# mozack/vdjer

Measured on AMD Instinct MI355X. Metric: M paired-reads/sec (k-mer build + contig score), IgH 50bp PE, higher is better.
Workload: dtype u8/u64 (2-bit packed bases, integer counts)

## Files before the change

vdjer_amd/csrc/vdjx_kmer.hip:

```cpp
#include "vdjx_common.h"

#include <algorithm>
#include <numeric>
#include <type_traits>
#include <string.h>
#include <stdlib.h>

#define HIST_THREADS 512
#define HIST_BLOCKS 512u
#define LOCAL_SLOTS 2048u
#define K3_SUB_TUPLES g_sub_tuples
__device__ u32 g_sub_tuples = 262144u;
#define NONE32 0xFFFFFFFFu
#define INST_MASK 0x7FFFFFFFu

struct RecView {
	u64 bhi, blo, nm, lq;
};

__device__ inline RecView load_rec(const u64* __restrict__ bases, const u64* __restrict__ nmask,
                                   const u64* __restrict__ lowq, size_t r) {
	RecView v;
	const ulonglong2 b = ((const ulonglong2*) bases)[r];
	v.bhi = b.x; v.blo = b.y;
// ... 425 lines not shown
	for (u32 i = threadIdx.x; i < nbk; i += 512) h[i] = 0;
	__syncthreads();
	const u32 seg = blockIdx.x / slices, sl = blockIdx.x % slices;
	const size_t s0 = seg_start[(size_t) seg << seg_shift], s1 = seg_start[((size_t) seg + 1) << seg_shift];
	const size_t per = (s1 - s0 + slices - 1) / slices;
	const size_t t0 = s0 + (size_t) sl * per;
	const size_t t1 = t0 + per < s1 ? t0 + per : s1;
	for (size_t t = t0 + threadIdx.x; t < t1; t += 512) {
		const TUP x = TUP::load(&in[t]);
		atomicAdd(&h[(u32) (vdjx_bucket_mix(x.lo, x.hi()) >> shift) & (nbk - 1)], 1u);
	}
	__syncthreads();
	for (u32 i = threadIdx.x; i < nbk; i += 512) if (h[i]) atomicAdd(&fine_cnt[((size_t) seg << sub_bits) | i], h[i]);
}

#ifndef RD_THREADS
#define RD_THREADS 768
#define RD_UNR 4
#define RD_WAVES 6
#endif
#define RD_SLOTS 2048u
#define RD_SLOT_BITS 11
#define RD_PQ 4096u
#define RD_LI 512u
#define RD_LROWS 128u
#define RD_MAXLOW 11u
#define ST_CAND 1u
#define ST_MULTI 2u
#define ST_QOK 4u
#define ST_QOK_R 8u
#define ST_ID_SHIFT 8
#define ST_NOID 0xFFFFFFu

struct SurvOutG { u64* lo; u64* hi; u32* gcnt; u64* gfirst; u32* n; u32 cap; u32* n_real; };
#define GC_SHADOW 0x80000000u
#define GC_MASK 0x7FFFFFFFu

__device__ inline bool reads_equal(const u64* __restrict__ bases, const u64* __restrict__ nmask, int rl, u64 a, u64 b) {
	if (rl <= VDJX_SHORT_READ_LEN) {
		const ulonglong2 x = ((const ulonglong2*) bases)[a];
		const ulonglong2 y = ((const ulonglong2*) bases)[b];
		return x.x == y.x && x.y == y.y && nmask[a] == nmask[b];
	}
	u64 d = 0;
#pragma unroll
	for (int w = 0; w < VDJX_LONG_W; w++) d |= bases[a * VDJX_LONG_W + w] ^ bases[b * VDJX_LONG_W + w];
#pragma unroll
	for (int w = 0; w < VDJX_LONG_M; w++) d |= nmask[a * VDJX_LONG_M + w] ^ nmask[b * VDJX_LONG_M + w];
// ... 28 lines not shown
		}
	}
	if (active) { c0 = atomicAdd(&cnt[idx], 1u); atomicMin((unsigned long long*) &mn[idx], (unsigned long long) val); }
	return c0;
}

__global__ __launch_bounds__(1024) void k_bucket_order(const u32* __restrict__ bucket_start, u32 NB, u32* __restrict__ order) {
	__shared__ u32 cls_cnt[33], cls_at[33];
	if (threadIdx.x < 33) cls_cnt[threadIdx.x] = 0;
	__syncthreads();
	for (u32 b = threadIdx.x; b < NB; b += 1024) {
		const u32 n = bucket_start[b + 1] - bucket_start[b];
		atomicAdd(&cls_cnt[n ? 32u - (u32) __builtin_clz(n) : 0u], 1u);
	}
	__syncthreads();
	if (threadIdx.x == 0) { u32 at = 0; for (int cl = 32; cl >= 0; cl--) { cls_at[cl] = at; at += cls_cnt[cl]; } }
	__syncthreads();
	for (u32 b = threadIdx.x; b < NB; b += 1024) {
		const u32 n = bucket_start[b + 1] - bucket_start[b];
		order[atomicAdd(&cls_at[n ? 32u - (u32) __builtin_clz(n) : 0u], 1u)] = b;
	}
}

template <typename TUP, bool SYM = false>
__global__ __launch_bounds__(RD_THREADS, sizeof(TUP) == 16 ? RD_WAVES : RD_WAVES / 2) void k_gated_reduce(const TUP* __restrict__ tup, const u32* __restrict__ bucket_start,
                                                             const u64* __restrict__ bases, const u64* __restrict__ nmask,
                                                             vdjx_qrows quals, int rl, int ob, int k, u64 rec_base,
                                                             u32 mf, u32 cmin, u32 mqq, u32 tlow, SurvOutG so,
                                                             u64* __restrict__ g_distinct, u32* __restrict__ g_err, u32 dbg_in,
                                                             const u32* __restrict__ order) {
#ifdef VDJX_ABLATE
	const u32 dbg = dbg_in;
#else
	const u32 dbg = dbg_in == 9u ? 9u : 0u;
#endif
	typedef typename TUP::hi_t THI;
	__shared__ u64 s_klo[RD_SLOTS];
	__shared__ THI s_khi[RD_SLOTS];
	__shared__ u64 s_first[RD_SLOTS];
	__shared__ u32 s_cnt[RD_SLOTS], s_state[RD_SLOTS];
	__shared__ u32 pq[RD_PQ];
	__shared__ u64 low_inst[RD_LI];
	__shared__ u32 low_n[RD_LROWS];
	__shared__ unsigned short low_slot[RD_LROWS];
	__shared__ u32 s_over, s_ndist, s_nlow, s_npq, s_nsurv, s_base, s_nreal;
	const THI EMPTY = (THI) ~(THI) 0;
	const u32 b = order ? order[blockIdx.x] : blockIdx.x;
	const u32 base = bucket_start[b];
	const u32 n = bucket_start[b + 1] - base;
	const u32 tid = threadIdx.x;
	if (n == 0) return;
	const TUP* T = tup + base;
	const u32 om = (1u << ob) - 1u;
	const u32 per_low = tlow > 1 ? (tlow - 1 < RD_MAXLOW ? tlow - 1 : RD_MAXLOW) : 1;
	const u32 lrows = RD_LI / per_low < RD_LROWS ? RD_LI / per_low : RD_LROWS;
	u32 S = 1;
	while ((u64) S * K3_SUB_TUPLES < n) S <<= 1;
	u32 ndist_total = 0;
	bool verify = S > 1;
	for (;;) {
		if (tid == 0) { s_over = 0; s_ndist = 0; }
		__syncthreads();
		for (u32 s = 0; s < S; s++) {
			for (u32 i = tid; i < RD_SLOTS; i += RD_THREADS) { s_khi[i] = EMPTY; s_cnt[i] = 0; s_first[i] = NONE64; s_state[i] = 0; }
			if (tid == 0) { s_nlow = 0; s_npq = (n >> (32 - RD_SLOT_BITS) || dbg == 9) ? RD_PQ + 1 : 0; s_nsurv = 0; s_nreal = 0; }
			__syncthreads();
			for (u32 t0 = 0; t0 < n; t0 += RD_UNR * RD_THREADS) {
				TUP r_t[RD_UNR];
#pragma unroll
				for (int j = 0; j < RD_UNR; j++) {
					const u32 t = t0 + j * RD_THREADS + tid;
					if (t < n) r_t[j] = TUP::load(&T[t]);
				}
#pragma unroll
				for (int j = 0; j < RD_UNR; j++) {
					const u32 t = t0 + j * RD_THREADS + tid;
					int slot = -1;
					if (t < n) {
						const u32 h = rd_hash(r_t[j].lo, r_t[j].hi());
						if (!(S > 1 && ((h >> 12) & (S - 1)) != s)) {
							slot = lds_insert<THI, RD_SLOTS>(s_klo, s_khi, r_t[j].lo, (THI) r_t[j].hi(), h);
							if (slot < 0) s_over = 1;
						}
					}
					const bool live = slot >= 0 && !verify;
					const u64 inst = r_t[j].inst();
					const u32 c0 = rd_count_min(s_cnt, s_first, (u32) (live ? slot : 0), inst, live);
					bool list = false;
					if (live) {
						u32 st = vdjx_peek(&s_state[slot]);
						if (!(st & ST_MULTI)) {
							const u64 f = vdjx_peek(&s_first[slot]);
							if (f != NONE64 && (f >> ob) != (inst >> ob)) {
								const u32 o1 = (u32) inst & om, o0 = (u32) f & om;
								const u32 d = o1 > o0 ? o1 - o0 : o0 - o1;
								if (d && d < (u32) k && !vdjx_kmer_has_period(r_t[j].hi(), r_t[j].lo, k, d)) { atomicOr(&s_state[slot], ST_MULTI); st |= ST_MULTI; }
							}
						}
						list = !((st & ST_MULTI) && c0 + 1 >= tlow);
					}
					const u32 qi = vdjx_wave_inc(&s_npq, list);
					if (list && qi < RD_PQ) pq[qi] = (t << RD_SLOT_BITS) | (u32) slot;
				}
			}
			__syncthreads();
			if (s_over || verify) { if (s_over) break; continue; }
			if (dbg == 1) return;
			for (u32 i = tid; i < RD_SLOTS; i += RD_THREADS) {
				if (s_khi[i] == EMPTY) continue;
				atomicAdd(&s_ndist, SYM ? 2u : 1u);
				const u32 c = s_cnt[i];
				if (c >= cmin) s_state[i] = (s_state[i] & ST_MULTI) | ST_CAND | ((c < tlow ? atomicAdd(&s_nlow, 1u) : ST_NOID) << ST_ID_SHIFT);
			}
			__syncthreads();
			const u32 nlow = s_nlow;
			const bool listed = s_npq <= RD_PQ;
			const u32 nscan = listed ? s_npq : n;
			for (u32 l0 = 0; l0 == 0 || l0 < nlow; l0 += lrows) {
				for (u32 i = tid; i < RD_LROWS; i += RD_THREADS) low_n[i] = 0;
				__syncthreads();
				for (u32 e = tid; e < nscan; e += RD_THREADS) {
					u32 slot, t;
					TUP x;
					if (listed) {
						slot = pq[e] & (RD_SLOTS - 1); t = pq[e] >> RD_SLOT_BITS;
						if (!(vdjx_peek(&s_state[slot]) & ST_CAND)) continue;
						x = TUP::load(&T[t]);
					} else {
						x = TUP::load(&T[e]);
						const u32 h = rd_hash(x.lo, x.hi());
						if (S > 1 && ((h >> 12) & (S - 1)) != s) continue;
						const int sl = lds_lookup<THI, RD_SLOTS>(s_klo, s_khi, x.lo, (THI) x.hi(), h);
						if (sl < 0) continue;
						slot = (u32) sl;
					}
					const u32 st = vdjx_peek(&s_state[slot]);
					if (!(st & ST_CAND)) continue;
					const u64 inst = x.inst(), fi = s_first[slot];
					const u32 lid = st >> ST_ID_SHIFT;
					if (lid != ST_NOID && lid >= l0 && lid < l0 + lrows) {
						const u32 pos = atomicAdd(&low_n[lid - l0], 1u);
						if (pos < per_low) low_inst[(lid - l0) * per_low + pos] = inst;
						low_slot[lid - l0] = (unsigned short) slot;
					}
					if (l0 == 0 && !(st & ST_MULTI) && (inst >> ob) != (fi >> ob)) {
						const u32 o1 = (u32) inst & om, o0 = (u32) fi & om;
						const u32 d = o1 > o0 ? o1 - o0 : o0 - o1;
						if ((d && d < (u32) k && !vdjx_kmer_has_period(x.hi(), x.lo, k, d))
						    || !reads_equal(bases, nmask, rl, (inst >> ob) - rec_base, (fi >> ob) - rec_base)) atomicOr(&s_state[slot], ST_MULTI);
					}
				}
				__syncthreads();
				if (dbg == 4) return;
				const u32 rows = nlow - l0 < lrows ? nlow - l0 : lrows;
				const u32 lane = tid & 63u;
				for (u32 r = tid >> 6; r < (nlow ? rows : 0u); r += RD_THREADS / 64) {
					const u32 slot = low_slot[r], cnt = low_n[r];
					const u64 fi = s_first[slot];
					u32 qv[RD_MAXLOW];
#pragma unroll
					for (u32 i = 0; i < RD_MAXLOW; i++) {
						qv[i] = 33u;
						if (i < cnt && i < per_low) {
							const u64 inst = low_inst[r * per_low + i];
							const uint8_t* q = quals.row((inst >> ob) - rec_base) + (inst == fi ? 0u : (u32) inst & om);
							if (lane < (u32) k) qv[i] = q[lane];
						}
					}
					u32 sum = 0;
#pragma unroll
					for (u32 i = 0; i < RD_MAXLOW; i++) sum += (u32) (uint8_t) (qv[i] - 33u);
					const bool lowq = lane < (u32) k && sum < mqq;
					if (!__ballot(lowq) && lane == 0) atomicOr(&s_state[slot], ST_QOK);
					if (SYM) {
						u64 fr = NONE64;
#pragma unroll
						for (u32 i = 0; i < RD_MAXLOW; i++)
							if (i < cnt && i < per_low) { const u64 m = vdjx_inst_mirror(low_inst[r * per_low + i], ob, rl, k); fr = m < fr ? m : fr; }
#pragma unroll
						for (u32 i = 0; i < RD_MAXLOW; i++) {
							qv[i] = 33u;
							if (i < cnt && i < per_low) {
								const u64 inst = vdjx_inst_mirror(low_inst[r * per_low + i], ob, rl, k);
								const uint8_t* q = quals.row((inst >> ob) - rec_base) + (inst == fr ? 0u : (u32) inst & om);
								if (lane < (u32) k) qv[i] = q[lane];
							}
						}
						u32 sum_r = 0;
#pragma unroll
						for (u32 i = 0; i < RD_MAXLOW; i++) sum_r += (u32) (uint8_t) (qv[i] - 33u);
						const bool lowq_r = lane < (u32) k && sum_r < mqq;
						if (!__ballot(lowq_r) && lane == 0) atomicOr(&s_state[slot], ST_QOK_R);
					}
				}
				__syncthreads();
			}
			if (dbg == 5) return;
			for (u32 i = tid; i < RD_SLOTS; i += RD_THREADS) {
				const u32 st = s_state[i];
				bool keep = false, keep_r = false;
				if (st & ST_CAND) {
					const u32 craw = s_cnt[i];
					const u32 c = craw > 32765u ? 32765u : craw;
					keep = c >= mf && (st & ST_MULTI) && (craw >= tlow || (st & ST_QOK));
					if (SYM) keep_r = c >= mf && (st & ST_MULTI) && (craw >= tlow || (st & ST_QOK_R));
				}
				if (SYM) {
					s_state[i] = (keep || keep_r) ? (atomicAdd(&s_nsurv, 2u) << 2) | (u32) keep | ((u32) keep_r << 1) : NONE32;
					if (keep || keep_r) atomicAdd(&s_nreal, (u32) keep + (u32) keep_r);
				} else s_state[i] = keep ? atomicAdd(&s_nsurv, 1u) : NONE32;
			}
			__syncthreads();
			if (tid == 0) { s_base = s_nsurv ? atomicAdd(so.n, s_nsurv) : 0; if (SYM && s_nreal) atomicAdd(so.n_real, s_nreal); }
			__syncthreads();
			for (u32 i = tid; i < RD_SLOTS; i += RD_THREADS) {
				if (s_state[i] == NONE32) continue;
				u32 pos = s_base + (SYM ? s_state[i] >> 2 : s_state[i]);
				const u32 cgo = s_cnt[i] > 32765u ? 32765u : s_cnt[i];
				if (pos < so.cap) {
					so.lo[pos] = s_klo[i];
					so.hi[pos] = (u64) s_khi[i];
					so.gcnt[pos] = cgo | (SYM && !(s_state[i] & 1u) ? GC_SHADOW : 0u);
					so.gfirst[pos] = s_first[i];
				}
				if (SYM) {
					pos += 1u;
					if (pos < so.cap) {
						u64 rh, rlo;
						vdjx_kmer_rc((u64) s_khi[i], s_klo[i], k, rh, rlo);
						so.lo[pos] = rlo;
						so.hi[pos] = rh;
						so.gcnt[pos] = cgo | (!(s_state[i] & 2u) ? GC_SHADOW : 0u);
						so.gfirst[pos] = vdjx_inst_mirror(s_first[i], ob, rl, k);
					}
				}
			}
			__syncthreads();
		}
// ... 545 lines not shown

__global__ void k_node_flags(const u64* __restrict__ s_lo, const u64* __restrict__ s_hi, u32 n, int k,
                             const u32* __restrict__ vbits, const u32* __restrict__ jbits,
                             uint8_t* __restrict__ has_v, uint8_t* __restrict__ has_j) {
	u32 i = blockIdx.x * blockDim.x + threadIdx.x;
	if (i >= n) return;
	if (k <= 16) { has_v[i] = 1; has_j[i] = 1; return; }
	u128 key = ((u128) s_hi[i] << 64) | s_lo[i];
	u32 code = (u32) (key >> (2 * (k - 16)));
	has_v[i] = code ? (vbits[code >> 5] >> (code & 31)) & 1u : 0;
	has_j[i] = code ? (jbits[code >> 5] >> (code & 31)) & 1u : 0;
}


#define IT_INST_BITS 35
#define IT_INST_MASK ((1ull << IT_INST_BITS) - 1ull)
#define IT_SURV_SHIFT 38
int vdjx_sort_pairs_raw(void* tmp, size_t* tmp_bytes, hipStream_t st, u64* k_in, u64* k_out, u32* v_in, u32* v_out, u32 n, unsigned end_bit);
#define IT_HOLE 0xFFFFFFFFFFFFFFFFull
#define WALK_THREADS 256

#define SLOT_HI_BITS 36
#define SLOT_HI_MASK ((1ull << SLOT_HI_BITS) - 1ull)
struct SurvTable { const ulonglong2* slots; u32 mask; const ulonglong2* skey; const u32* bloom; u32 bloom_mask; };

struct ItemFmt {
	u32 pmask;
	u32 len_shift;
	u32 maxlen;
	u32 mul, inv;
	u32 bmask;
	u32 ns;
};
__device__ inline u32 it_surv(const ItemFmt& f, u64 x) { return (u32) (x >> IT_SURV_SHIFT) & f.pmask; }
__device__ inline u32 it_len(const ItemFmt& f, u64 x) { return f.maxlen > 1 ? (u32) (x >> f.len_shift) + 1u : 1u; }
__device__ inline u32 it_scat(const ItemFmt& f, u32 p) { return ((((p >> 4) * f.mul) & f.bmask) << 4) | (p & 15u); }

__global__ void k_surv_table2(const u64* __restrict__ s_lo, const u64* __restrict__ s_hi, u32 n, ulonglong2* __restrict__ slots, u32 mask,
                              ulonglong2* __restrict__ skey, u32* __restrict__ bloom, u32 bloom_mask) {
	const u32 i = blockIdx.x * blockDim.x + threadIdx.x;
	if (i >= n) return;
	const u64 lo = s_lo[i], hi = s_hi[i];
	skey[i] = make_ulonglong2(lo, hi);
	const u64 h = vdjx_mix(lo, hi);
	{
		const u32 bit = (u32) (h >> 40) & bloom_mask;
		atomicOr(&bloom[bit >> 5], 1u << (bit & 31));
	}
	u32 slot = (u32) (h >> 20) & mask;
	const unsigned long long entry = hi | ((unsigned long long) (i + 1) << SLOT_HI_BITS);
	while (atomicCAS((unsigned long long*) &slots[slot].y, 0ull, entry) != 0ull) slot = (slot + 1) & mask;
	slots[slot].x = lo;
}

__device__ inline int surv_lookup2f(const SurvTable& t, u64 lo, u64 hi);

__device__ inline int surv_lookup2(const SurvTable& t, u64 lo, u64 hi) {
	u32 slot = (u32) (vdjx_mix(lo, hi) >> 20) & t.mask;
	for (;;) {
		const ulonglong2 v = t.slots[slot];
		if (!v.y) return -1;
		if (v.x == lo && (v.y & SLOT_HI_MASK) == hi) return (int) (v.y >> SLOT_HI_BITS) - 1;
		slot = (slot + 1) & t.mask;
	}
}

__device__ inline int surv_lookup2f(const SurvTable& t, u64 lo, u64 hi) {
	const u64 h = vdjx_mix(lo, hi);
	const u32 bit = (u32) (h >> 40) & t.bloom_mask;
	if (!((t.bloom[bit >> 5] >> (bit & 31)) & 1u)) return -1;
	return surv_lookup2(t, lo, hi);
}

__global__ void k_succ_links2(SurvTable t, u32 n, int k, const u32* __restrict__ gcnt, u32* __restrict__ succ, unsigned long long* __restrict__ pred,
                              u32* __restrict__ bestsucc) {
	const u32 u = blockIdx.x * blockDim.x + threadIdx.x;
	if (u >= n) return;
	const ulonglong2 kk = t.skey[u];
	const u128 base = (((u128) kk.y << 64) | kk.x) << 2;
	const u128 km = k < 64 ? (((u128) 1) << (2 * k)) - 1 : ~(u128) 0;
	const int sh = 2 * (k - 1);
	const u32 fb = (u32) (sh < 64 ? kk.x >> sh : kk.y >> (sh - 64)) & 3u;
	const unsigned long long mine = ((unsigned long long) (gcnt[u] & GC_MASK) << 32) | ((unsigned long long) (fb ^ 1u) << 30) | (unsigned long long) u;
	u32 best = NONE32, best_g = 0;
	for (u32 b = 0; b < 4; b++) {
		const u128 key = (base | (u128) b) & km;
		const int s = surv_lookup2(t, (u64) key, (u64) (key >> 64));
		succ[u * 4 + b] = s >= 0 ? (u32) s : NONE32;
		if (s >= 0 && (u32) s != u) {
			const u32 g = gcnt[s] & GC_MASK;
			if (best == NONE32 || g >= best_g) { best = (u32) s; best_g = g; }
			atomicMax(&pred[s], mine);
// ... 260 lines not shown
				if (lm) {
					if (later) {
						const u32 qi = qn + (u32) __popcll(lm & ((1ull << lane) - 1ull));
						dq[wq][qi] = ((u64) r << 8) | (u64) (u32) o;
						if constexpr (!LONG) { dq_b[wq][qi] = make_ulonglong2(v.bhi, v.blo); dq_v[wq][qi] = V; }
						o = P; need = false;
					}
					qn += (u32) __popcll(lm);
				}
			}
			WST(if (__ballot(need)) st_lookup++;)
			if (!FRESH && __ballot(need && !first && !have_c)) {
				WST(st_filter++;)
				const bool mine = need && !first && !have_c;
				for (int ob = 0; ob < P; ob += 4) {
					u32 wv[4], bt[4];
#pragma unroll
					for (int j = 0; j < 4; j++) {
						const int oo = ob + j;
						wv[j] = 0; bt[j] = 0;
						if (mine && oo >= o && oo < P && wm_test(V, oo)) {
							u64 khi, klo;
							v.kmer_u(k, oo, khi, klo);
							const u32 bit = (u32) (vdjx_mix(klo, khi) >> 40) & t.bloom_mask;
							bt[j] = bit & 31u;
							wv[j] = (dbg & 8u) ? 0xFFFFFFFFu : t.bloom[bit >> 5];
						}
					}
#pragma unroll
					for (int j = 0; j < 4; j++) if ((wv[j] >> bt[j]) & 1u) wm_set(C, ob + j);
				}
				if (mine) have_c = true;
			}
			if (need) {
				bool filtered = false;
				if (!first) {
					o = wm_next(C, o, P);
					filtered = true;
				}
				first = false;
				if (o < P) {
					u64 khi, klo;
					v.kmer_l(k, o, khi, klo);
					if (dbg & 8u) s = (klo & 3u) ? (int) ((u32) vdjx_mix(klo, khi) % f.ns) : -1;
					else s = (filtered || (dbg & 16u)) ? surv_lookup2(t, klo, khi) : surv_lookup2f(t, klo, khi);
					in = 0;
					if (s < 0) o++;
// ... 473 lines not shown
	for (int e = 0; e < 4; e++) { o.from_ids[(size_t) r * 4 + e] = f[e] != NONE64 ? id[e] : 0; deg += f[e] != NONE64; }
	o.from_deg[r] = (uint8_t) deg;
}

namespace {

struct PersistAlloc {
	vdjx_ctx* c;
	explicit PersistAlloc(vdjx_ctx* ctx) : c(ctx) {}
	template <typename T> hipError_t alloc(T** out, size_t n) {
		*out = (T*) c->shard_arena.alloc((n ? n : 1) * sizeof(T));
		return *out ? hipSuccess : hipErrorOutOfMemory;
	}
	vdjx_arena::mark_t mark() const { return c->shard_arena.mark(); }
	void release_to(vdjx_arena::mark_t m) { c->shard_arena.release_to(m); }
};

struct PoolView { const u64* bases; const u64* nmask; vdjx_qrows quals; int rl; int ob; };

template <typename TUP> struct GTuples {
	TUP* t = nullptr;
	u32* bucket_start = nullptr;
	u32 NB = 0, N = 0;
};

struct SurvivorsG {
	u64 *lo = nullptr, *hi = nullptr, *gfirst = nullptr, *ufirst = nullptr;
	u32 *gcnt = nullptr, *ucnt = nullptr;
	u32 n = 0, n_real = 0;
	u64 ndist = 0;
};

inline u32 ceil_log2_u64(u64 x) { u32 b = 0; while ((1ull << b) < x) b++; return b; }

static bool sync_debug() { static const bool on = vdjx_env_set("VDJX_SYNC_DEBUG"); return on; }
static void dbg_sync(vdjx_ctx* c, const char* what) {
	if (!sync_debug()) return;
	const hipError_t e = hipStreamSynchronize(c->stream);
	fprintf(stderr, "[vdjx] %s: %s\n", what, hipGetErrorString(e));
}

struct GatedHist { u32 HB = 0, NBH = 0, N = 0; u32* hstart = nullptr; bool sym = false; };
static bool build_sym(const vdjx_pool* pool, int k) {
	return pool->sym && pool->W == 2 && (k & 1) && pool->n_records % 2 == 0;
}
static bool sym_walk_wanted() { static const bool on = !vdjx_env_set("VDJX_NO_SYM_WALK"); return on; }
static size_t gated_bucket_default() { static const size_t v = (size_t) vdjx_env_num("VDJX_GATED_BUCKET", 3072, 1, 1ll << 32); return v; }
template <typename A>
int stage_gated_hist(vdjx_ctx* c, A& db, const vdjx_pool* pool, int k, size_t per_bucket, u64 geometry_instances, GatedHist* gh, bool sym = false) {
	hipStream_t st = c->stream;
	const size_t R = sym ? pool->n_records / 2 : pool->n_records;
	const int P = pool->rl - k + 1;
	const u64 NI = geometry_instances ? geometry_instances : (u64) R * (u64) P;
	const size_t per = per_bucket ? per_bucket : gated_bucket_default();
	const u32 hb_max = pool->W > 2 ? 14u : 15u;
	u32 HB = ceil_log2_u64((NI + per - 1) / per);
	HB = std::max(8u, std::min(hb_max, HB));
	const u32 NBH = 1u << HB;
#ifdef VDJX_ABLATE
	static const u32 hist_dbg = (u32) vdjx_env_num("VDJX_HIST_DBG", 0, 0, 4);
#else
	constexpr u32 hist_dbg = 0;
#endif
	u32 nblk = (u32) std::min<size_t>(HIST_BLOCKS, (R + 4095) / 4096);
	if (nblk == 0) nblk = 1;
	size_t rpb = (R + nblk - 1) / nblk;
	u32 *hcnt, *hstart;
	HIP_TRY(db.alloc(&hcnt, NBH));
	HIP_TRY(db.alloc(&hstart, NBH + 1));
	HIP_TRY(hipMemsetAsync(hcnt, 0, (size_t) NBH * 4, st));
	const bool lng = pool->W > 2;
	const size_t lds_hist = (size_t) NBH * 4 + (HIST_THREADS / 64) * (lng ? GL_WAVE_BYTES_LONG : GL_WAVE_BYTES);
	HIP_TRY(hipFuncSetAttribute((const void*) k_gated_hist<false>, hipFuncAttributeMaxDynamicSharedMemorySize, (int) lds_hist));
	HIP_TRY(hipFuncSetAttribute((const void*) k_gated_hist<true>, hipFuncAttributeMaxDynamicSharedMemorySize, (int) lds_hist));
	HIP_TRY(hipFuncSetAttribute((const void*) k_gated_hist<false, true>, hipFuncAttributeMaxDynamicSharedMemorySize, (int) lds_hist));
	{
		vdjx_prof_scope ps(c, "k_gated_hist");
// ... 11 lines not shown
#endif
	const u32 N = *(const u32*) c->h_pin;
	c->stats["gated_instances"] = sym ? 2ull * N : N;
	gh->HB = HB; gh->NBH = NBH; gh->N = N; gh->hstart = hstart; gh->sym = sym;
	return VDJX_OK;
}

template <typename TUP, typename A>
int stage_gated_cut(vdjx_ctx* c, A& db, const vdjx_pool* pool, u64 rec_base, int k, size_t per_bucket, u64 geometry_instances, const GatedHist& gh, GTuples<TUP>* out) {
	hipStream_t st = c->stream;
	const bool sym = gh.sym;
	const size_t R = sym ? pool->n_records / 2 : pool->n_records;
	const int P = pool->rl - k + 1;
	const size_t per = per_bucket ? per_bucket : gated_bucket_default();
	const u32 hb_max = pool->W > 2 ? 14u : 15u;
	const bool lng = pool->W > 2;
	const u32 HB = gh.HB, NBH = gh.NBH, N = gh.N;
	u32* hstart = gh.hstart;
	size_t rpb;
	out->N = N;
	const u64 Ng = geometry_instances ? geometry_instances : (u64) N;
	static const size_t refine = (size_t) vdjx_env_num("VDJX_REFINE_TUPLES", 4096, 1, 1ll << 32);
	u32 T = 8;
	while (T < HB && ((u64) per << T) < Ng) T++;
	u32 extra = 0;
	const size_t refine_at = per_bucket ? std::max<size_t>(per_bucket, refine / 2) : refine;
	if (T == HB && HB == hb_max && Ng / NBH > refine_at) {
		extra = 1;
		while (extra < 5 && (Ng >> extra) / NBH > refine_at) extra++;
	}
	const u32 Tt = T + extra;
	const u32 NBt = 1u << Tt;
	HIP_TRY(db.alloc(&out->t, (size_t) N + 1));
	constexpr u32 stage_tuples = PARTR_STAGE_BYTES / (u32) sizeof(TUP);
	constexpr u32 lds_partr = PARTR_STAGE_BYTES + stage_tuples * 4;
	HIP_TRY(hipFuncSetAttribute((const void*) k_part_records_g<TUP, false>, hipFuncAttributeMaxDynamicSharedMemorySize, (int) lds_partr));
	HIP_TRY(hipFuncSetAttribute((const void*) k_part_records_g<TUP, true>, hipFuncAttributeMaxDynamicSharedMemorySize, (int) lds_partr));
	HIP_TRY(hipFuncSetAttribute((const void*) k_part_records_g<TUP, false, true>, hipFuncAttributeMaxDynamicSharedMemorySize, (int) lds_partr));
	HIP_TRY(hipFuncSetAttribute((const void*) k_part_tuples_g<TUP>, hipFuncAttributeMaxDynamicSharedMemorySize, PART_LDS_BYTES));
	u32 cbits = Tt, fbits = 0;
	if (Tt > 10) { cbits = extra ? Tt - 10 : 8; fbits = Tt - cbits; }
	const u32 NBc = 1u << cbits;
	u32 nblk2 = (u32) std::min<size_t>(1024, (R + 2047) / 2048);
	if (nblk2 == 0) nblk2 = 1;
	rpb = (R + nblk2 - 1) / nblk2;
	u32* gcur;
	HIP_TRY(db.alloc(&gcur, NBc));
	TUP* l1 = out->t;
	if (fbits) HIP_TRY(db.alloc(&l1, (size_t) N + 1));
	{
		vdjx_prof_scope ps(c, "k_part_records");
		hipLaunchKernelGGL(k_init_cursors, dim3((NBc + 255) / 256), dim3(256), 0, st, hstart, NBc, HB - cbits, gcur);
		const u64 NIl = (u64) R * (u64) P;
		u64 rr = N ? (u64) stage_tuples * 3 / 4 * NIl / ((u64) N * (u64) P) : 1u << 16;
// ... 58 lines not shown
}

template <typename TUP, typename A>
int stage_gated_reduce(vdjx_ctx* c, A& db, const GTuples<TUP>& t, const PoolView& pv, u64 rec_base, int k, int mf, int mq, SurvivorsG* sv, bool sym = false) {
	hipStream_t st = c->stream;
	int rc = set_sub_tuples(c);
	if (rc) return rc;
	if (mq >= 255) mq = 254;
	const u32 mqq = (u32) (mq < 0 ? 0 : (mq > 214 ? 214 : mq));
	const u32 tlow = 1 + (mqq + 19) / 20;
	const u32 cmin = (u32) std::max(mf, 2);
	const u32 mfu = (u32) std::max(mf, 0);
	const u32 cap = (sym ? t.N : t.N / 2) + 16;
	u32 *g_err, *n_surv;
	u64* g_distinct;
	HIP_TRY(db.alloc(&sv->lo, cap)); HIP_TRY(db.alloc(&sv->hi, cap)); HIP_TRY(db.alloc(&sv->gcnt, cap)); HIP_TRY(db.alloc(&sv->gfirst, cap));
	HIP_TRY(db.alloc(&g_distinct, 64 * 16 + 2));
	g_err = (u32*) (g_distinct + 64 * 16);
	n_surv = g_err + 1;
	u32* n_real = g_err + 2;
	HIP_TRY(hipMemsetAsync(g_distinct, 0, (64 * 16 + 2) * 8, st));
	SurvOutG so{sv->lo, sv->hi, sv->gcnt, sv->gfirst, n_surv, cap, n_real};
	static const u32 rd_dbg = (u32) vdjx_env_num("VDJX_RD_DBG", 0, 0, 9);
	if (t.N) {
		vdjx_prof_scope ps(c, "k_gated_reduce");
		u32* order;
		if ((rc = bucket_order(c, db, t, &order))) return rc;
		if (sym) hipLaunchKernelGGL((k_gated_reduce<TUP, true>), dim3(t.NB), dim3(RD_THREADS), 0, st, t.t, t.bucket_start, pv.bases, pv.nmask, pv.quals, pv.rl, pv.ob, k, rec_base,
		                            mfu, cmin, mqq, tlow, so, g_distinct, g_err, rd_dbg, (const u32*) order);
		else hipLaunchKernelGGL(k_gated_reduce<TUP>, dim3(t.NB), dim3(RD_THREADS), 0, st, t.t, t.bucket_start, pv.bases, pv.nmask, pv.quals, pv.rl, pv.ob, k, rec_base,
		                        mfu, cmin, mqq, tlow, so, g_distinct, g_err, rd_dbg, (const u32*) order);
	}
	u64* spread = (u64*) c->h_pin;
	u32* tail = (u32*) (spread + 64 * 16);
	static_assert((64 * 16 + 2) * 8 == VDJX_HPIN_SYNC_BYTES, "h_pin layout (vdjx_common.h)");
	HIP_TRY(hipMemcpyAsync(spread, g_distinct, VDJX_HPIN_SYNC_BYTES, hipMemcpyDeviceToHost, st));
	HIP_TRY(hipStreamSynchronize(st));
	HIP_TRY(hipGetLastError());
	const u32 ns = tail[1], err = tail[0];
	if (err) { vdjx_set_error("k_gated_reduce: %u buckets could not be split to fit LDS", err); return VDJX_EHIP; }
	if (ns > cap) { vdjx_set_error("survivor capacity logic failed (%u > %u)", ns, cap); return VDJX_EHIP; }
	sv->ndist = 0;
	for (int i = 0; i < 64; i++) sv->ndist += spread[i * 16];
	sv->n = ns;
	sv->n_real = sym ? tail[2] : ns;
	c->stats["kmer_build_shadows"] = ns - sv->n_real;
	return VDJX_OK;
}

struct RecountOut { u32* ucnt; u64* ufirst; u64* in_first; u32* in_from; u64* edge_first; u32* edge_to; };
struct RecountStatus { const u32* g_err = nullptr; const u32* n_items = nullptr; const unsigned long long* n_inst = nullptr; u32 ns = 0; };
#define VDJX_ESYMWALK (-1000)
static int recount_status_check(vdjx_ctx* c, const u32* hp, u32 ns) {
	if (hp[6] || hp[7]) { vdjx_set_error("the mirrored walk found %u + %u places where the chains are not mirror images", hp[6], hp[7]); return VDJX_ESYMWALK; }
	if (hp[0]) { vdjx_set_error("k_walk_items: item buffer too small (%u waves stopped)", hp[0]); return VDJX_EHIP; }
	if (hp[1]) { vdjx_set_error("internal error: %u of %u surviving k-mers were not met again in the records (VDJX_SYNC_DEBUG=1 names them)", hp[1], ns); return VDJX_EHIP; }
	c->stats["recount_items"] = hp[2];
	c->stats["recount_instances"] = *(const unsigned long long*) (hp + 4);
	return VDJX_OK;
}

template <typename A>
int stage_recount(vdjx_ctx* c, A& db, const vdjx_pool* pool, u64 rec_base, int k, SurvivorsG& sv, const RecountOut& ro,
                  bool derive_edges, SurvTable* table_out = nullptr, RecountStatus* defer = nullptr, bool sym_walk = false) {
	hipStream_t st = c->stream;
	const size_t R = pool->n_records;
	const int P = pool->rl - k + 1;
	const u32 ns = sv.n;
	if (ns >= (1u << 26)) { vdjx_set_error("more than 2^26 surviving k-mers: not supported by the recount items"); return VDJX_ELIMIT; }
	if (R >= (1ull << 29)) { vdjx_set_error("more than 2^29 records on one GPU: not supported by the recount items"); return VDJX_ELIMIT; }
	if ((u64) R * (u64) P >= (1ull << 32)) { vdjx_set_error("records*offsets = %llu >= 2^32 on one GPU: shard the pool over more GPUs", (unsigned long long) ((u64) R * (u64) P)); return VDJX_ELIMIT; }
	u32 tmask = 1023;
	while ((size_t) tmask + 1 < (size_t) ns * 2) tmask = tmask * 2 + 1;
	unsigned long long* pred;
	ulonglong2* table;
	u32 *succ0, *succ, *bloom, *clen, *coff, *csum, *csum_start, *newidx, *jump_open, *fbw, *gcnt2, *bestsucc, *partner = nullptr;
	u64 *pd, *lo2, *hi2, *gfirst2, *linw;
	ulonglong2 *skey0, *skey;
	u32 bloom_bits = 1u << 16;
	while (bloom_bits < (1u << 30) && (size_t) bloom_bits < (size_t) ns * 16) bloom_bits <<= 1;
	const u32 nb16 = (ns + 15u) >> 4;
	const u32 n_scan = (ns + SCAN_BLOCK - 1) / SCAN_BLOCK;
	const u32 n_jump = (ceil_log2_u64((u64) ns + 1) + 4) / 5 + 1;
	{
		auto up = [](size_t b) { return (b + 255) & ~(size_t) 255; };
		const size_t b_bloom = up(bloom_bits / 8), b_table = up(((size_t) tmask + 1) * 16), b_pred = up((size_t) ns * 8), b_clen = up((size_t) ns * 4),
		             b_jump = up((size_t) (n_jump + 1) * 4), b_linw = up(((size_t) nb16 + 1) * 8);
		uint8_t* z;
		const size_t zb = b_bloom + b_table + b_pred + b_clen + b_jump + b_linw;
		HIP_TRY(db.alloc(&z, zb));
		HIP_TRY(hipMemsetAsync(z, 0, zb, st));
		table = (ulonglong2*) z; z += b_table;
		bloom = (u32*) z; z += b_bloom;
		pred = (unsigned long long*) z; z += b_pred;
		clen = (u32*) z; z += b_clen;
		jump_open = (u32*) z; z += b_jump;
		linw = (u64*) z;
	}
	HIP_TRY(db.alloc(&skey0, ns)); HIP_TRY(db.alloc(&skey, ns));
	HIP_TRY(db.alloc(&succ0, (size_t) ns * 4)); HIP_TRY(db.alloc(&succ, (size_t) ns * 4));
	HIP_TRY(db.alloc(&pd, ns)); HIP_TRY(db.alloc(&coff, ns));
	HIP_TRY(db.alloc(&csum, n_scan)); HIP_TRY(db.alloc(&csum_start, n_scan + 1)); HIP_TRY(db.alloc(&newidx, ns));
	HIP_TRY(db.alloc(&lo2, ns)); HIP_TRY(db.alloc(&hi2, ns)); HIP_TRY(db.alloc(&gcnt2, ns)); HIP_TRY(db.alloc(&gfirst2, ns));
	HIP_TRY(db.alloc(&fbw, nb16));
	HIP_TRY(db.alloc(&bestsucc, ns));
	if (sym_walk) HIP_TRY(db.alloc(&partner, ns));
	const SurvTable tb0{table, tmask, skey0, bloom, bloom_bits - 1};
	const SurvTable tb{table, tmask, skey, bloom, bloom_bits - 1};
	if (table_out) *table_out = tb;
	const dim3 gs((ns + 255) / 256), bs(256);
	{
		vdjx_prof_scope ps(c, "k_surv_table");
		hipLaunchKernelGGL(k_surv_table2, gs, bs, 0, st, sv.lo, sv.hi, ns, table, tmask, skey0, bloom, bloom_bits - 1);
		hipLaunchKernelGGL(k_succ_links2, gs, bs, 0, st, tb0, ns, k, sv.gcnt, succ0, pred, bestsucc);
	}
	{
		vdjx_prof_scope ps(c, "k_chain_order");
		hipLaunchKernelGGL(k_chain_init, gs, bs, 0, st, pred, bestsucc, ns, pd);
		for (u32 j = 0; j < n_jump; j++) hipLaunchKernelGGL(k_chain_jump, gs, bs, 0, st, pd, ns, j ? jump_open + j - 1 : (const u32*) nullptr, jump_open + j);
		hipLaunchKernelGGL(k_chain_len, gs, bs, 0, st, pd, ns, clen);
		hipLaunchKernelGGL(k_scan_sums, dim3(n_scan), dim3(256), 0, st, clen, ns, csum);
		hipLaunchKernelGGL(k_bucket_scan, dim3(1), dim3(1024), 0, st, csum, n_scan, csum_start);
		hipLaunchKernelGGL(k_scan_apply, dim3(n_scan), dim3(256), 0, st, clen, ns, csum_start, coff);
		hipLaunchKernelGGL(k_chain_place, gs, bs, 0, st, pd, coff, ns, newidx);
		hipLaunchKernelGGL(k_chain_permute, gs, bs, 0, st, newidx, ns, sv.lo, sv.hi, sv.gcnt, sv.gfirst, succ0, lo2, hi2, gcnt2, gfirst2, skey, succ);
		hipLaunchKernelGGL(k_table_remap, dim3(tmask / 256 + 1), bs, 0, st, table, tmask + 1, newidx);
		if (sym_walk) hipLaunchKernelGGL(k_partner, gs, bs, 0, st, tb, ns, k, partner);
		hipLaunchKernelGGL(k_chain_words, gs, bs, 0, st, succ, skey, ns, k, linw, fbw, (const u32*) partner);
	}
	dbg_sync(c, "k_chain_order");
	if (sync_debug()) {
		std::vector<u32> ni(ns), seen(ns, 0);
		(void) hipMemcpy(ni.data(), newidx, (size_t) ns * 4, hipMemcpyDeviceToHost);
		u32 dup = 0, oob = 0;
		for (u32 i = 0; i < ns; i++) { if (ni[i] >= ns) oob++; else if (seen[ni[i]]++) dup++; }
		std::vector<u64> pdh(ns);
		std::vector<unsigned long long> prh(ns);
		(void) hipMemcpy(pdh.data(), pd, (size_t) ns * 8, hipMemcpyDeviceToHost);
		(void) hipMemcpy(prh.data(), pred, (size_t) ns * 8, hipMemcpyDeviceToHost);
		u32 unresolved = 0;
		for (u32 i = 0; i < ns; i++) { const u32 p0 = (u32) (pdh[i] >> 32); if (p0 != NONE32 && (u32) (pdh[p0] >> 32) != NONE32) unresolved++; }
		fprintf(stderr, "[vdjx] chain order: %u survivors, %u duplicate new indices, %u out of range, %u unresolved (cycles), %u jump launches\n", ns, dup, oob, unresolved, n_jump);
		for (u32 i = 0, shown = 0; i < ns && shown < 6; i++) if (ni[i] < ns && seen[ni[i]] > 1) {
			fprintf(stderr, "[vdjx]   old %u -> new %u: pd = (%u, %u), pred word %llx\n", i, ni[i], (u32) (pdh[i] >> 32), (u32) pdh[i], prh[i]);
			shown++;
		}
	}
	sv.lo = lo2; sv.hi = hi2; sv.gcnt = gcnt2; sv.gfirst = gfirst2;
	ItemFmt f;
// ... 944 lines not shown
```

Before: 908.4.

## Add small-bucket gated reduce geometry and size survivor hash table exactly

Templates k_gated_reduce over slot count, thread count and queue size, and adds a small configuration (1024 slots, 384 threads) that is chosen automatically when buckets hold about 1.5K tuples, with more buckets made to match. The smaller LDS footprint lets more blocks share a CU and cuts the per-bucket cost of clearing and scanning the table. The survivor hash table and bloom filter now use multiply-shift range reduction instead of power-of-two masks, so they can be sized exactly at about 2x and 16x the survivor count rather than rounded up. This lowers memory footprint and cache pressure, at the cost of a multiply per probe and a wrap compare in place of a mask.

After: 885.6. -2.5%, worse.

```diff
diff --git a/vdjer_amd/csrc/vdjx_kmer.hip b/vdjer_amd/csrc/vdjx_kmer.hip
--- a/vdjer_amd/csrc/vdjx_kmer.hip
+++ b/vdjer_amd/csrc/vdjx_kmer.hip
@@ -471,8 +471,11 @@
 #define RD_SLOTS 2048u
 #define RD_SLOT_BITS 11
 #define RD_PQ 4096u
-#define RD_LI 512u
-#define RD_LROWS 128u
+#define RDS_THREADS 384
+#define RDS_SLOTS 1024u
+#define RDS_SLOT_BITS 10
+#define RDS_PQ 2048u
+#define RDS_MAX_TUPLES 2048u
 #define RD_MAXLOW 11u
 #define ST_CAND 1u
 #define ST_MULTI 2u
@@ -547,8 +550,8 @@
 	}
 }
 
-template <typename TUP, bool SYM = false>
-__global__ __launch_bounds__(RD_THREADS, sizeof(TUP) == 16 ? RD_WAVES : RD_WAVES / 2) void k_gated_reduce(const TUP* __restrict__ tup, const u32* __restrict__ bucket_start,
+template <typename TUP, bool SYM = false, u32 SLOTS = RD_SLOTS, u32 THREADS = RD_THREADS, u32 PQ = RD_PQ, u32 SLOT_BITS = RD_SLOT_BITS>
+__global__ __launch_bounds__(THREADS, sizeof(TUP) == 16 ? RD_WAVES : RD_WAVES / 2) void k_gated_reduce(const TUP* __restrict__ tup, const u32* __restrict__ bucket_start,
                                                              const u64* __restrict__ bases, const u64* __restrict__ nmask,
                                                              vdjx_qrows quals, int rl, int ob, int k, u64 rec_base,
                                                              u32 mf, u32 cmin, u32 mqq, u32 tlow, SurvOutG so,
@@ -560,14 +563,16 @@
 	const u32 dbg = dbg_in == 9u ? 9u : 0u;
 #endif
 	typedef typename TUP::hi_t THI;
-	__shared__ u64 s_klo[RD_SLOTS];
-	__shared__ THI s_khi[RD_SLOTS];
-	__shared__ u64 s_first[RD_SLOTS];
-	__shared__ u32 s_cnt[RD_SLOTS], s_state[RD_SLOTS];
-	__shared__ u32 pq[RD_PQ];
-	__shared__ u64 low_inst[RD_LI];
-	__shared__ u32 low_n[RD_LROWS];
-	__shared__ unsigned short low_slot[RD_LROWS];
+	constexpr u32 LI = SLOTS / 4, LROWS = SLOTS / 16;
+	static_assert(SLOTS == (1u << SLOT_BITS) && THREADS % 64 == 0 && SLOTS <= 65536u, "list entries carry the slot in SLOT_BITS bits, low_slot[] in 16");
+	__shared__ u64 s_klo[SLOTS];
+	__shared__ THI s_khi[SLOTS];
+	__shared__ u64 s_first[SLOTS];
+	__shared__ u32 s_cnt[SLOTS], s_state[SLOTS];
+	__shared__ u32 pq[PQ];
+	__shared__ u64 low_inst[LI];
+	__shared__ u32 low_n[LROWS];
+	__shared__ unsigned short low_slot[LROWS];
 	__shared__ u32 s_over, s_ndist, s_nlow, s_npq, s_nsurv, s_base, s_nreal;
 	const THI EMPTY = (THI) ~(THI) 0;
 	const u32 b = order ? order[blockIdx.x] : blockIdx.x;
@@ -578,7 +583,7 @@
 	const TUP* T = tup + base;
 	const u32 om = (1u << ob) - 1u;
 	const u32 per_low = tlow > 1 ? (tlow - 1 < RD_MAXLOW ? tlow - 1 : RD_MAXLOW) : 1;
-	const u32 lrows = RD_LI / per_low < RD_LROWS ? RD_LI / per_low : RD_LROWS;
+	const u32 lrows = LI / per_low < LROWS ? LI / per_low : LROWS;
 	u32 S = 1;
 	while ((u64) S * K3_SUB_TUPLES < n) S <<= 1;
 	u32 ndist_total = 0;
@@ -587,24 +592,24 @@
 		if (tid == 0) { s_over = 0; s_ndist = 0; }
 		__syncthreads();
 		for (u32 s = 0; s < S; s++) {
-			for (u32 i = tid; i < RD_SLOTS; i += RD_THREADS) { s_khi[i] = EMPTY; s_cnt[i] = 0; s_first[i] = NONE64; s_state[i] = 0; }
-			if (tid == 0) { s_nlow = 0; s_npq = (n >> (32 - RD_SLOT_BITS) || dbg == 9) ? RD_PQ + 1 : 0; s_nsurv = 0; s_nreal = 0; }
+			for (u32 i = tid; i < SLOTS; i += THREADS) { s_khi[i] = EMPTY; s_cnt[i] = 0; s_first[i] = NONE64; s_state[i] = 0; }
+			if (tid == 0) { s_nlow = 0; s_npq = (n >> (32 - SLOT_BITS) || dbg == 9) ? PQ + 1 : 0; s_nsurv = 0; s_nreal = 0; }
 			__syncthreads();
-			for (u32 t0 = 0; t0 < n; t0 += RD_UNR * RD_THREADS) {
+			for (u32 t0 = 0; t0 < n; t0 += RD_UNR * THREADS) {
 				TUP r_t[RD_UNR];
 #pragma unroll
 				for (int j = 0; j < RD_UNR; j++) {
-					const u32 t = t0 + j * RD_THREADS + tid;
+					const u32 t = t0 + j * THREADS + tid;
 					if (t < n) r_t[j] = TUP::load(&T[t]);
 				}
 #pragma unroll
 				for (int j = 0; j < RD_UNR; j++) {
-					const u32 t = t0 + j * RD_THREADS + tid;
+					const u32 t = t0 + j * THREADS + tid;
 					int slot = -1;
 					if (t < n) {
 						const u32 h = rd_hash(r_t[j].lo, r_t[j].hi());
 						if (!(S > 1 && ((h >> 12) & (S - 1)) != s)) {
-							slot = lds_insert<THI, RD_SLOTS>(s_klo, s_khi, r_t[j].lo, (THI) r_t[j].hi(), h);
+							slot = lds_insert<THI, SLOTS>(s_klo, s_khi, r_t[j].lo, (THI) r_t[j].hi(), h);
 							if (slot < 0) s_over = 1;
 						}
 					}
@@ -625,13 +630,13 @@
 						list = !((st & ST_MULTI) && c0 + 1 >= tlow);
 					}
 					const u32 qi = vdjx_wave_inc(&s_npq, list);
-					if (list && qi < RD_PQ) pq[qi] = (t << RD_SLOT_BITS) | (u32) slot;
+					if (list && qi < PQ) pq[qi] = (t << SLOT_BITS) | (u32) slot;
 				}
 			}
 			__syncthreads();
 			if (s_over || verify) { if (s_over) break; continue; }
 			if (dbg == 1) return;
-			for (u32 i = tid; i < RD_SLOTS; i += RD_THREADS) {
+			for (u32 i = tid; i < SLOTS; i += THREADS) {
 				if (s_khi[i] == EMPTY) continue;
 				atomicAdd(&s_ndist, SYM ? 2u : 1u);
 				const u32 c = s_cnt[i];
@@ -639,23 +644,23 @@
 			}
 			__syncthreads();
 			const u32 nlow = s_nlow;
-			const bool listed = s_npq <= RD_PQ;
+			const bool listed = s_npq <= PQ;
 			const u32 nscan = listed ? s_npq : n;
 			for (u32 l0 = 0; l0 == 0 || l0 < nlow; l0 += lrows) {
-				for (u32 i = tid; i < RD_LROWS; i += RD_THREADS) low_n[i] = 0;
+				for (u32 i = tid; i < LROWS; i += THREADS) low_n[i] = 0;
 				__syncthreads();
-				for (u32 e = tid; e < nscan; e += RD_THREADS) {
+				for (u32 e = tid; e < nscan; e += THREADS) {
 					u32 slot, t;
 					TUP x;
 					if (listed) {
-						slot = pq[e] & (RD_SLOTS - 1); t = pq[e] >> RD_SLOT_BITS;
+						slot = pq[e] & (SLOTS - 1); t = pq[e] >> SLOT_BITS;
 						if (!(vdjx_peek(&s_state[slot]) & ST_CAND)) continue;
 						x = TUP::load(&T[t]);
 					} else {
 						x = TUP::load(&T[e]);
 						const u32 h = rd_hash(x.lo, x.hi());
 						if (S > 1 && ((h >> 12) & (S - 1)) != s) continue;
-						const int sl = lds_lookup<THI, RD_SLOTS>(s_klo, s_khi, x.lo, (THI) x.hi(), h);
+						const int sl = lds_lookup<THI, SLOTS>(s_klo, s_khi, x.lo, (THI) x.hi(), h);
 						if (sl < 0) continue;
 						slot = (u32) sl;
 					}
@@ -679,7 +684,7 @@
 				if (dbg == 4) return;
 				const u32 rows = nlow - l0 < lrows ? nlow - l0 : lrows;
 				const u32 lane = tid & 63u;
-				for (u32 r = tid >> 6; r < (nlow ? rows : 0u); r += RD_THREADS / 64) {
+				for (u32 r = tid >> 6; r < (nlow ? rows : 0u); r += THREADS / 64) {
 					const u32 slot = low_slot[r], cnt = low_n[r];
 					const u64 fi = s_first[slot];
 					u32 qv[RD_MAXLOW];
@@ -721,7 +726,7 @@
 				__syncthreads();
 			}
 			if (dbg == 5) return;
-			for (u32 i = tid; i < RD_SLOTS; i += RD_THREADS) {
+			for (u32 i = tid; i < SLOTS; i += THREADS) {
 				const u32 st = s_state[i];
 				bool keep = false, keep_r = false;
 				if (st & ST_CAND) {
@@ -738,7 +743,7 @@
 			__syncthreads();
 			if (tid == 0) { s_base = s_nsurv ? atomicAdd(so.n, s_nsurv) : 0; if (SYM && s_nreal) atomicAdd(so.n_real, s_nreal); }
 			__syncthreads();
-			for (u32 i = tid; i < RD_SLOTS; i += RD_THREADS) {
+			for (u32 i = tid; i < SLOTS; i += THREADS) {
 				if (s_state[i] == NONE32) continue;
 				u32 pos = s_base + (SYM ? s_state[i] >> 2 : s_state[i]);
 				const u32 cgo = s_cnt[i] > 32765u ? 32765u : s_cnt[i];
@@ -1330,7 +1335,9 @@
 
 #define SLOT_HI_BITS 36
 #define SLOT_HI_MASK ((1ull << SLOT_HI_BITS) - 1ull)
-struct SurvTable { const ulonglong2* slots; u32 mask; const ulonglong2* skey; const u32* bloom; u32 bloom_mask; };
+struct SurvTable { const ulonglong2* slots; u32 n_slots; const ulonglong2* skey; const u32* bloom; u32 n_bits; };
+__device__ inline u32 surv_slot(u64 h, u32 n_slots) { return (u32) (((u64) (u32) h * n_slots) >> 32); }
+__device__ inline u32 surv_bit(u64 h, u32 n_bits) { return (u32) (((h >> 32) * n_bits) >> 32); }
 
 struct ItemFmt {
 	u32 pmask;
@@ -1344,38 +1351,38 @@
 __device__ inline u32 it_len(const ItemFmt& f, u64 x) { return f.maxlen > 1 ? (u32) (x >> f.len_shift) + 1u : 1u; }
 __device__ inline u32 it_scat(const ItemFmt& f, u32 p) { return ((((p >> 4) * f.mul) & f.bmask) << 4) | (p & 15u); }
 
-__global__ void k_surv_table2(const u64* __restrict__ s_lo, const u64* __restrict__ s_hi, u32 n, ulonglong2* __restrict__ slots, u32 mask,
-                              ulonglong2* __restrict__ skey, u32* __restrict__ bloom, u32 bloom_mask) {
+__global__ void k_surv_table2(const u64* __restrict__ s_lo, const u64* __restrict__ s_hi, u32 n, ulonglong2* __restrict__ slots, u32 n_slots,
+                              ulonglong2* __restrict__ skey, u32* __restrict__ bloom, u32 n_bits) {
 	const u32 i = blockIdx.x * blockDim.x + threadIdx.x;
 	if (i >= n) return;
 	const u64 lo = s_lo[i], hi = s_hi[i];
 	skey[i] = make_ulonglong2(lo, hi);
 	const u64 h = vdjx_mix(lo, hi);
 	{
-		const u32 bit = (u32) (h >> 40) & bloom_mask;
+		const u32 bit = surv_bit(h, n_bits);
 		atomicOr(&bloom[bit >> 5], 1u << (bit & 31));
 	}
-	u32 slot = (u32) (h >> 20) & mask;
+	u32 slot = surv_slot(h, n_slots);
 	const unsigned long long entry = hi | ((unsigned long long) (i + 1) << SLOT_HI_BITS);
-	while (atomicCAS((unsigned long long*) &slots[slot].y, 0ull, entry) != 0ull) slot = (slot + 1) & mask;
+	while (atomicCAS((unsigned long long*) &slots[slot].y, 0ull, entry) != 0ull) slot = slot + 1 == n_slots ? 0u : slot + 1;
 	slots[slot].x = lo;
 }
 
 __device__ inline int surv_lookup2f(const SurvTable& t, u64 lo, u64 hi);
 
 __device__ inline int surv_lookup2(const SurvTable& t, u64 lo, u64 hi) {
-	u32 slot = (u32) (vdjx_mix(lo, hi) >> 20) & t.mask;
+	u32 slot = surv_slot(vdjx_mix(lo, hi), t.n_slots);
 	for (;;) {
 		const ulonglong2 v = t.slots[slot];
 		if (!v.y) return -1;
 		if (v.x == lo && (v.y & SLOT_HI_MASK) == hi) return (int) (v.y >> SLOT_HI_BITS) - 1;
-		slot = (slot + 1) & t.mask;
+		slot = slot + 1 == t.n_slots ? 0u : slot + 1;
 	}
 }
 
 __device__ inline int surv_lookup2f(const SurvTable& t, u64 lo, u64 hi) {
 	const u64 h = vdjx_mix(lo, hi);
-	const u32 bit = (u32) (h >> 40) & t.bloom_mask;
+	const u32 bit = surv_bit(h, t.n_bits);
 	if (!((t.bloom[bit >> 5] >> (bit & 31)) & 1u)) return -1;
 	return surv_lookup2(t, lo, hi);
 }
@@ -1682,7 +1689,7 @@
 						if (mine && oo >= o && oo < P && wm_test(V, oo)) {
 							u64 khi, klo;
 							v.kmer_u(k, oo, khi, klo);
-							const u32 bit = (u32) (vdjx_mix(klo, khi) >> 40) & t.bloom_mask;
+							const u32 bit = surv_bit(vdjx_mix(klo, khi), t.n_bits);
 							bt[j] = bit & 31u;
 							wv[j] = (dbg & 8u) ? 0xFFFFFFFFu : t.bloom[bit >> 5];
 						}
@@ -2202,6 +2209,7 @@
 	TUP* t = nullptr;
 	u32* bucket_start = nullptr;
 	u32 NB = 0, N = 0;
+	bool small = false;
 };
 
 struct SurvivorsG {
@@ -2226,13 +2234,18 @@
 }
 static bool sym_walk_wanted() { static const bool on = !vdjx_env_set("VDJX_NO_SYM_WALK"); return on; }
 static size_t gated_bucket_default() { static const size_t v = (size_t) vdjx_env_num("VDJX_GATED_BUCKET", 3072, 1, 1ll << 32); return v; }
+#define RDS_AIM_TUPLES 1536u
+static bool gated_bucket_auto(size_t per_bucket, u64 geometry_instances, int k) {
+	static const bool named = vdjx_env_set("VDJX_GATED_BUCKET");
+	return !per_bucket && !named && !geometry_instances && k <= 45;
+}
 template <typename A>
 int stage_gated_hist(vdjx_ctx* c, A& db, const vdjx_pool* pool, int k, size_t per_bucket, u64 geometry_instances, GatedHist* gh, bool sym = false) {
 	hipStream_t st = c->stream;
 	const size_t R = sym ? pool->n_records / 2 : pool->n_records;
 	const int P = pool->rl - k + 1;
 	const u64 NI = geometry_instances ? geometry_instances : (u64) R * (u64) P;
-	const size_t per = per_bucket ? per_bucket : gated_bucket_default();
+	const size_t per = gated_bucket_auto(per_bucket, geometry_instances, k) ? RDS_AIM_TUPLES : per_bucket ? per_bucket : gated_bucket_default();
 	const u32 hb_max = pool->W > 2 ? 14u : 15u;
 	u32 HB = ceil_log2_u64((NI + per - 1) / per);
 	HB = std::max(8u, std::min(hb_max, HB));
@@ -2290,14 +2303,23 @@
 	const u64 Ng = geometry_instances ? geometry_instances : (u64) N;
 	static const size_t refine = (size_t) vdjx_env_num("VDJX_REFINE_TUPLES", 4096, 1, 1ll << 32);
 	u32 T = 8;
-	while (T < HB && ((u64) per << T) < Ng) T++;
+	bool small = false;
+	if (gated_bucket_auto(per_bucket, geometry_instances, k)) {
+		while (T < HB && ((u64) RDS_AIM_TUPLES << T) < Ng) T++;
+		small = ((u64) RDS_AIM_TUPLES << T) >= Ng;
+		if (!small) T = 8;
+	}
+	if (!small) while (T < HB && ((u64) per << T) < Ng) T++;
 	u32 extra = 0;
 	const size_t refine_at = per_bucket ? std::max<size_t>(per_bucket, refine / 2) : refine;
-	if (T == HB && HB == hb_max && Ng / NBH > refine_at) {
+	if (!small && T == HB && HB == hb_max && Ng / NBH > refine_at) {
 		extra = 1;
 		while (extra < 5 && (Ng >> extra) / NBH > refine_at) extra++;
+		if (gated_bucket_auto(per_bucket, geometry_instances, k) && extra < 5 && (Ng >> (extra + 1)) / NBH <= RDS_MAX_TUPLES) { extra++; small = true; }
 	}
 	const u32 Tt = T + extra;
+	if (!gated_bucket_auto(per_bucket, geometry_instances, k)) small = !geometry_instances && sizeof(TUP) == 16 && (Ng >> Tt) <= RDS_MAX_TUPLES;
+	out->small = small;
 	const u32 NBt = 1u << Tt;
 	HIP_TRY(db.alloc(&out->t, (size_t) N + 1));
 	constexpr u32 stage_tuples = PARTR_STAGE_BYTES / (u32) sizeof(TUP);
@@ -2402,12 +2424,21 @@
 	HIP_TRY(hipMemsetAsync(g_distinct, 0, (64 * 16 + 2) * 8, st));
 	SurvOutG so{sv->lo, sv->hi, sv->gcnt, sv->gfirst, n_surv, cap, n_real};
 	static const u32 rd_dbg = (u32) vdjx_env_num("VDJX_RD_DBG", 0, 0, 9);
+	c->stats["gated_reduce_slots"] = t.small ? RDS_SLOTS : RD_SLOTS;
 	if (t.N) {
 		vdjx_prof_scope ps(c, "k_gated_reduce");
 		u32* order;
 		if ((rc = bucket_order(c, db, t, &order))) return rc;
-		if (sym) hipLaunchKernelGGL((k_gated_reduce<TUP, true>), dim3(t.NB), dim3(RD_THREADS), 0, st, t.t, t.bucket_start, pv.bases, pv.nmask, pv.quals, pv.rl, pv.ob, k, rec_base,
-		                            mfu, cmin, mqq, tlow, so, g_distinct, g_err, rd_dbg, (const u32*) order);
+		if (t.small) {
+			if constexpr (sizeof(TUP) == 16) {
+				if (sym) hipLaunchKernelGGL((k_gated_reduce<TUP, true, RDS_SLOTS, RDS_THREADS, RDS_PQ, RDS_SLOT_BITS>), dim3(t.NB), dim3(RDS_THREADS), 0, st, t.t, t.bucket_start, pv.bases, pv.nmask, pv.quals,
+				                            pv.rl, pv.ob, k, rec_base, mfu, cmin, mqq, tlow, so, g_distinct, g_err, rd_dbg, (const u32*) order);
+				else hipLaunchKernelGGL((k_gated_reduce<TUP, false, RDS_SLOTS, RDS_THREADS, RDS_PQ, RDS_SLOT_BITS>), dim3(t.NB), dim3(RDS_THREADS), 0, st, t.t, t.bucket_start, pv.bases, pv.nmask, pv.quals,
+				                        pv.rl, pv.ob, k, rec_base, mfu, cmin, mqq, tlow, so, g_distinct, g_err, rd_dbg, (const u32*) order);
+			} else { vdjx_set_error("k_gated_reduce: the small geometry takes 16-byte tuples only"); return VDJX_ESTATE; }
+		}
+		else if (sym) hipLaunchKernelGGL((k_gated_reduce<TUP, true>), dim3(t.NB), dim3(RD_THREADS), 0, st, t.t, t.bucket_start, pv.bases, pv.nmask, pv.quals, pv.rl, pv.ob, k, rec_base,
+		                                 mfu, cmin, mqq, tlow, so, g_distinct, g_err, rd_dbg, (const u32*) order);
 		else hipLaunchKernelGGL(k_gated_reduce<TUP>, dim3(t.NB), dim3(RD_THREADS), 0, st, t.t, t.bucket_start, pv.bases, pv.nmask, pv.quals, pv.rl, pv.ob, k, rec_base,
 		                        mfu, cmin, mqq, tlow, so, g_distinct, g_err, rd_dbg, (const u32*) order);
 	}
@@ -2450,21 +2481,21 @@
 	if (ns >= (1u << 26)) { vdjx_set_error("more than 2^26 surviving k-mers: not supported by the recount items"); return VDJX_ELIMIT; }
 	if (R >= (1ull << 29)) { vdjx_set_error("more than 2^29 records on one GPU: not supported by the recount items"); return VDJX_ELIMIT; }
 	if ((u64) R * (u64) P >= (1ull << 32)) { vdjx_set_error("records*offsets = %llu >= 2^32 on one GPU: shard the pool over more GPUs", (unsigned long long) ((u64) R * (u64) P)); return VDJX_ELIMIT; }
-	u32 tmask = 1023;
-	while ((size_t) tmask + 1 < (size_t) ns * 2) tmask = tmask * 2 + 1;
+	const u32 n_slots = std::max<u32>(1024u, (2u * ns + 7u) & ~7u);
 	unsigned long long* pred;
 	ulonglong2* table;
 	u32 *succ0, *succ, *bloom, *clen, *coff, *csum, *csum_start, *newidx, *jump_open, *fbw, *gcnt2, *bestsucc, *partner = nullptr;
 	u64 *pd, *lo2, *hi2, *gfirst2, *linw;
 	ulonglong2 *skey0, *skey;
-	u32 bloom_bits = 1u << 16;
-	while (bloom_bits < (1u << 30) && (size_t) bloom_bits < (size_t) ns * 16) bloom_bits <<= 1;
+	const u32 bloom_bits = std::max<u32>(1u << 16, (16u * ns + 31u) & ~31u);
+	c->stats["surv_table_slots"] = n_slots;
+	c->stats["surv_filter_bits"] = bloom_bits;
 	const u32 nb16 = (ns + 15u) >> 4;
 	const u32 n_scan = (ns + SCAN_BLOCK - 1) / SCAN_BLOCK;
 	const u32 n_jump = (ceil_log2_u64((u64) ns + 1) + 4) / 5 + 1;
 	{
 		auto up = [](size_t b) { return (b + 255) & ~(size_t) 255; };
-		const size_t b_bloom = up(bloom_bits / 8), b_table = up(((size_t) tmask + 1) * 16), b_pred = up((size_t) ns * 8), b_clen = up((size_t) ns * 4),
+		const size_t b_bloom = up(bloom_bits / 8), b_table = up((size_t) n_slots * 16), b_pred = up((size_t) ns * 8), b_clen = up((size_t) ns * 4),
 		             b_jump = up((size_t) (n_jump + 1) * 4), b_linw = up(((size_t) nb16 + 1) * 8);
 		uint8_t* z;
 		const size_t zb = b_bloom + b_table + b_pred + b_clen + b_jump + b_linw;
@@ -2485,13 +2516,13 @@
 	HIP_TRY(db.alloc(&fbw, nb16));
 	HIP_TRY(db.alloc(&bestsucc, ns));
 	if (sym_walk) HIP_TRY(db.alloc(&partner, ns));
-	const SurvTable tb0{table, tmask, skey0, bloom, bloom_bits - 1};
-	const SurvTable tb{table, tmask, skey, bloom, bloom_bits - 1};
+	const SurvTable tb0{table, n_slots, skey0, bloom, bloom_bits};
+	const SurvTable tb{table, n_slots, skey, bloom, bloom_bits};
 	if (table_out) *table_out = tb;
 	const dim3 gs((ns + 255) / 256), bs(256);
 	{
 		vdjx_prof_scope ps(c, "k_surv_table");
-		hipLaunchKernelGGL(k_surv_table2, gs, bs, 0, st, sv.lo, sv.hi, ns, table, tmask, skey0, bloom, bloom_bits - 1);
+		hipLaunchKernelGGL(k_surv_table2, gs, bs, 0, st, sv.lo, sv.hi, ns, table, n_slots, skey0, bloom, bloom_bits);
 		hipLaunchKernelGGL(k_succ_links2, gs, bs, 0, st, tb0, ns, k, sv.gcnt, succ0, pred, bestsucc);
 	}
 	{
@@ -2504,7 +2535,7 @@
 		hipLaunchKernelGGL(k_scan_apply, dim3(n_scan), dim3(256), 0, st, clen, ns, csum_start, coff);
 		hipLaunchKernelGGL(k_chain_place, gs, bs, 0, st, pd, coff, ns, newidx);
 		hipLaunchKernelGGL(k_chain_permute, gs, bs, 0, st, newidx, ns, sv.lo, sv.hi, sv.gcnt, sv.gfirst, succ0, lo2, hi2, gcnt2, gfirst2, skey, succ);
-		hipLaunchKernelGGL(k_table_remap, dim3(tmask / 256 + 1), bs, 0, st, table, tmask + 1, newidx);
+		hipLaunchKernelGGL(k_table_remap, dim3((n_slots + 255) / 256), bs, 0, st, table, n_slots, newidx);
 		if (sym_walk) hipLaunchKernelGGL(k_partner, gs, bs, 0, st, tb, ns, k, partner);
 		hipLaunchKernelGGL(k_chain_words, gs, bs, 0, st, succ, skey, ns, k, linw, fbw, (const u32*) partner);
 	}
```
